# likojack/bnv_fusion

Hardware: AMD Instinct MI355X
Metric: depth frames/sec fused+decoded, 640x480 @ 256^3 grid (higher is better)
Workload: dtype f32 operands split into f16 hi+lo, 3 products on v_mfma_f32_16x16x32_f16, f32 accumulate

## Files before the change

### bnv_fusion_amd/csrc/encode.hip

```cpp
#include <stddef.h>

#include <atomic>
#include <utility>
#include <vector>

#include "frontend.hpp"
#include "tcnn_mlp.hpp"

namespace bnv {

int g_num_cus = 0;
int g_last_hip_error = 0;
std::atomic<int> g_reserve_cus{0};
std::atomic<int> g_finalize_blocks{0};
std::atomic<int> g_tcnn_shared_table{1};
std::atomic<int> g_tcnn_block_encoder{1};
std::atomic<int> g_mlp_mode{1};

bool g_prof_on = false;
static std::vector<std::pair<hipEvent_t, hipEvent_t>> g_prof_events[PROF_KINDS];
static size_t g_prof_used[PROF_KINDS] = {0, 0, 0, 0};

void prof_mark(int kind, bool begin, hipStream_t stream) {
  auto& ring = g_prof_events[kind];
// ... 651 lines not shown
  const int64_t n = ctl->n_deferred;
  const int nyz = g.n_xyz[1] * g.n_xyz[2];
  for (int64_t q = (int64_t)blockIdx.x * 256 + threadIdx.x; q < n; q += (int64_t)gridDim.x * 256) {
    const int id = ids[defer_list[q]];
    const int x = id / nyz, r = id - x * nyz, y = r / g.n_xyz[2], z = r - y * g.n_xyz[2];
    if (shard_is_boundary(x, y, z, g)) atomicAdd(&s_hist[voxel_owner(x, y, z, g) & 63], 1);
  }
  __syncthreads();
  if (threadIdx.x < 64 && threadIdx.x < g.shard_world && s_hist[threadIdx.x])
    atomicAdd(&ctl->shard_boundary[threadIdx.x], s_hist[threadIdx.x]);
}

struct ValidFlags {
  const int32_t* counts;
  const int32_t* ids;
  bnv_grid_t g;
  int emit_all;
  __device__ uint32_t operator()(int64_t s) const {
    if (!emit_all && counts[s] < g.min_pts_in_grid) return 0;
    if (g.shard_world > 1) {
      const int id = ids[s];
      const int nyz = g.n_xyz[1] * g.n_xyz[2];
      const int x = id / nyz, r = id - x * nyz, y = r / g.n_xyz[2], z = r - y * g.n_xyz[2];
      if (voxel_owner(x, y, z, g) != g.shard_rank) return 0;
    }
    return 1;
  }
};

struct PairTiles {
  const int32_t* list;
  int n_pairs, n_points, n_pblocks, n_tiles;
};
__device__ __forceinline__ PairTiles pair_tiles(int n_points, const int32_t* __restrict__ pair_list,
                                                const int32_t* __restrict__ n_pairs) {
  PairTiles T;
  T.list = pair_list;
  T.n_points = n_points;
  T.n_pblocks = (n_points + 31) >> 5;
  T.n_pairs = pair_list ? *n_pairs : 0;
  T.n_tiles = pair_list ? (T.n_pairs + 31) >> 5 : T.n_pblocks * 8;
  return T;
}
__device__ __forceinline__ bool tile_pair(const PairTiles& T, int t, int j, int* i, int* k) {
  if (T.list) {
    const int e = t * 32 + j;
    if (e >= T.n_pairs) return false;
    const int p = T.list[e];
    *i = p >> 3;
    *k = p & 7;
    return true;
  }
  *k = t / T.n_pblocks;
  *i = (t - *k * T.n_pblocks) * 32 + j;
  return *i < T.n_points;
}

__device__ __forceinline__ f32x16 relu16(f32x16 v) {
#pragma unroll
  for (int r = 0; r < 16; ++r) v[r] = relu_bits(v[r]);
  return v;
}

__device__ __forceinline__ f32x16 bias_init(const float* __restrict__ b, int mb, int h) {
  f32x16 v;
#pragma unroll
  for (int q = 0; q < 4; ++q) {
    const f32x4 t = *(const f32x4*)&b[mb * 32 + 8 * q + 4 * h];
#pragma unroll
    for (int i = 0; i < 4; ++i) v[4 * q + i] = t[i];
  }
  return v;
}

__device__ __forceinline__ void layer128(const float* __restrict__ wp, const float* __restrict__ bias,
                                         const f32x16 (&in)[4], f32x16 (&out)[4], int lane, int h) {
#pragma unroll
  for (int mb = 0; mb < 4; ++mb) out[mb] = bias_init(bias, mb, h);
#pragma unroll
  for (int nb = 0; nb < 4; ++nb) {
#pragma unroll
    for (int rq = 0; rq < 4; ++rq) {
      f32x4 a[4];
#pragma unroll
      for (int mb = 0; mb < 4; ++mb)
        a[mb] = *(const f32x4*)&wp[(((mb * 4 + nb) * 4 + rq) * 64 + lane) * 4];
#pragma unroll
// ... 50 lines not shown
    if (s > 0) v[q] -= ((unsigned long long)phi << 32) | plo;
  }
}

__device__ __forceinline__ void scatter_tile(const f32x16& o, int slot, int j, int h, int32_t* __restrict__ counts,
                                             long long* __restrict__ acc) {
  unsigned long long v[4];
  bool is_end;
  int len;
  tile_run_sums(o, slot, j, h, v, is_end, len);
#ifdef BNV_PROBE_NO_SCATTER
  if ((blockIdx.x & 63) != 0) return;
#endif
  if (slot >= 0 && is_end) {
    unsigned long long* dst = (unsigned long long*)acc + ((uint32_t)slot * 8u + 4u * (uint32_t)h);
#pragma unroll
    for (int q = 0; q < 4; ++q) atomicAdd(dst + q, v[q]);
    if (h == 0) atomicAdd(&counts[slot], len);
  }
}

__global__ __launch_bounds__(512, 2) void k_pointnet_scatter(
    const float* __restrict__ pts, int n_points, bnv_grid_t g, const float* __restrict__ wpack,
    const uint32_t* __restrict__ bitmap, const uint32_t* __restrict__ word_prefix,
    int32_t* __restrict__ counts, long long* __restrict__ acc, const int32_t* __restrict__ pair_list,
    const int32_t* __restrict__ n_pairs) {
  extern __shared__ __attribute__((aligned(16))) float lds[];
  stage_to_lds<512>(wpack, lds, PN_TOTAL * 4);
  __syncthreads();

  const int lane = threadIdx.x & 63;
  const int wave = __builtin_amdgcn_readfirstlane(threadIdx.x >> 6);
  const int j = lane & 31, h = lane >> 5;
  const PairTiles T = pair_tiles(n_points, pair_list, n_pairs);
  const int n_tiles = T.n_tiles;
  const int nyz = g.n_xyz[1] * g.n_xyz[2];

  for (int t = blockIdx.x * 8 + wave; t < n_tiles; t += gridDim.x * 8) {
    int i = 0, k = 0;
    const bool have = tile_pair(T, t, j, &i, &k);
    float in0 = 0.f, in1 = 0.f, in2 = 0.f;
    int slot = -1;
    bool valid = false;
    if (have) {
      const float* p = pts + (size_t)i * 6;
      const float x = p[0], y = p[1], z = p[2];
      valid = in_bounds(x, y, z, g);
      if (valid) {
        const float xn = voxel_coord(x, g.bound_min[0], g.voxel_size);
        const float yn = voxel_coord(y, g.bound_min[1], g.voxel_size);
        const float zn = voxel_coord(z, g.bound_min[2], g.voxel_size);
        const int gx = (k & 1) ? (int)ceilf(xn) : (int)floorf(xn);
        const int gy = (k & 2) ? (int)ceilf(yn) : (int)floorf(yn);
        const int gz = (k & 4) ? (int)ceilf(zn) : (int)floorf(zn);
        if (voxel_owner(gx, gy, gz, g) == g.shard_rank) {
          const uint32_t id = (uint32_t)(gx * nyz + gy * g.n_xyz[2] + gz);
          const uint32_t word = bitmap[id >> 5];
          slot = (int)(word_prefix[id >> 5] + __popc(word & ((1u << (id & 31)) - 1u)));
        }
        const float rx = relative_coord(xn, gx, g.voxel_size);
        const float ry = relative_coord(yn, gy, g.voxel_size);
        const float rz = relative_coord(zn, gz, g.voxel_size);
        in0 = h ? ry : rx;
        in1 = h ? p[3] : rz;
        in2 = h ? p[5] : p[4];
      }
    }
    if (__ballot(slot >= 0) == 0ULL) continue;

    f32x16 ha[4], hb[4];
#pragma unroll
    for (int mb = 0; mb < 4; ++mb) ha[mb] = bias_init(lds + PN_B1, mb, h);
    {
// ... 12 lines not shown
#pragma unroll
    for (int mb = 0; mb < 4; ++mb) hb[mb] = relu16(hb[mb]);
    layer128(lds + PN_W3, lds + PN_B3, hb, ha, lane, h);
#pragma unroll
    for (int mb = 0; mb < 4; ++mb) ha[mb] = relu16(ha[mb]);
    f32x16 o;
#pragma unroll
    for (int r = 0; r < 16; ++r) o[r] = 0.f;
    {
      const f32x4 b4 = *(const f32x4*)&lds[PN_B4 + 4 * h];
#pragma unroll
      for (int r = 0; r < 4; ++r) o[r] = b4[r];
    }
#pragma unroll
    for (int nb = 0; nb < 4; ++nb) {
#pragma unroll
      for (int rq = 0; rq < 4; ++rq) {
        f32x4 a = {0.f, 0.f, 0.f, 0.f};
        if (j < 8) a = *(const f32x4*)&lds[PN_W4 + ((((nb * 4 + rq) * 2 + h) * 8) + j) * 4];
#pragma unroll
        for (int i = 0; i < 4; ++i)
          o = __builtin_amdgcn_mfma_f32_32x32x2f32(a[i], ha[nb][4 * rq + i], o, 0, 0, 0);
      }
    }
    scatter_tile(o, slot, j, h, counts, acc);
  }
}


typedef __attribute__((address_space(3))) const half8 lds_half8_t;
typedef __attribute__((address_space(3))) const f32x4 lds_f32x4_t;
constexpr int kLdsWin = 61440;

#ifdef BNV_PHASE_PROF
__device__ unsigned long long g_enc_phase[8 * 16];
#define BNV_EPH(i)                                                                          \
  do {                                                                                      \
    if ((threadIdx.x & 63) == 0) {                                                          \
      unsigned long long* _p = (unsigned long long*)((char*)lds + PX_LDS_BYTES) + (threadIdx.x >> 6) * 16; \
      const unsigned long long _t = clock64();                                              \
      _p[i] += _t - _p[15];                                                                 \
      _p[15] = _t;                                                                          \
    }                                                                                       \
  } while (0)
constexpr int kEncProfLds = 8 * 16 * 8;
#else
#define BNV_EPH(i)
constexpr int kEncProfLds = 0;
#endif

struct EncLdsX {
  uint32_t w[3];
  uint32_t b;
};
__device__ __forceinline__ half8 ldsx_wfrag(const EncLdsX& L, int byte_off) {
  const int b = byte_off / kLdsWin;
  return *(lds_half8_t*)((b == 0 ? L.w[0] : (b == 1 ? L.w[1] : L.w[2])) + (uint32_t)(byte_off - b * kLdsWin));
}
__device__ __forceinline__ f32x4 ldsx_bias(const EncLdsX& L, int layer, int rb) {
  return *(lds_f32x4_t*)(L.b + (uint32_t)((layer * 128 + rb * 16) * 4));
}

template <int NPROD>
__device__ __forceinline__ void layer128_x(const EncLdsX& L, int w_off, int layer, const half8 (&inh)[4][2],
                                           const half8 (&inl)[4][2], f32x4 (&out)[8][2]) {
#pragma unroll
  for (int rb = 0; rb < 8; ++rb) out[rb][0] = out[rb][1] = ldsx_bias(L, layer, rb);
  half8 ah[2], al[2];
#define BNV_LOAD_WX(q)                                                        \
  {                                                                           \
    const int wb = (w_off + (q) * 2 * 64 * 8) * 2;                            \
    ah[(q) & 1] = ldsx_wfrag(L, wb);                                          \
    if (NPROD == 3) al[(q) & 1] = ldsx_wfrag(L, wb + 1024);                   \
  }
  BNV_LOAD_WX(0);
#pragma unroll
  for (int q = 0; q < 32; ++q) {
    if (q + 1 < 32) BNV_LOAD_WX(q + 1);
    __builtin_amdgcn_sched_barrier(0);
    const int s = q >> 3, rb = q & 7;
    if constexpr (NPROD == 3) {
      out[rb][0] = __builtin_amdgcn_mfma_f32_16x16x32_f16(al[q & 1], inh[s][0], out[rb][0], 0, 0, 0);
      out[rb][1] = __builtin_amdgcn_mfma_f32_16x16x32_f16(al[q & 1], inh[s][1], out[rb][1], 0, 0, 0);
      out[rb][0] = __builtin_amdgcn_mfma_f32_16x16x32_f16(ah[q & 1], inl[s][0], out[rb][0], 0, 0, 0);
      out[rb][1] = __builtin_amdgcn_mfma_f32_16x16x32_f16(ah[q & 1], inl[s][1], out[rb][1], 0, 0, 0);
    }
    out[rb][0] = __builtin_amdgcn_mfma_f32_16x16x32_f16(ah[q & 1], inh[s][0], out[rb][0], 0, 0, 0);
    out[rb][1] = __builtin_amdgcn_mfma_f32_16x16x32_f16(ah[q & 1], inh[s][1], out[rb][1], 0, 0, 0);
    __builtin_amdgcn_sched_barrier(0);
  }
#undef BNV_LOAD_WX
}

template <int NPROD>
__device__ __forceinline__ void split_x(const f32x4 (&acc)[8][2], half8 (&oh)[4][2], half8 (&ol)[4][2]) {
#pragma unroll
  for (int s = 0; s < 4; ++s)
#pragma unroll
    for (int cb = 0; cb < 2; ++cb) {
      float x[8];
#pragma unroll
      for (int e = 0; e < 8; ++e) x[e] = relu_bits(acc[2 * s + (e >> 2)][cb][e & 3]);
      if (NPROD == 3) {
        split8_f16(x, oh[s][cb], ol[s][cb]);
      } else {
#pragma unroll
        for (int e = 0; e < 8; ++e) oh[s][cb][e] = (_Float16)x[e];
      }
    }
}

__device__ __forceinline__ void scatter_tile_x(const f32x4& o, int slot, int n, int g, int32_t* __restrict__ counts,
                                               long long* __restrict__ acc) {
  uint32_t lo[4], hi[4];
#pragma unroll
  for (int q = 0; q < 4; ++q) {
    const float r = __builtin_rintf(o[q] * kFixedScale);
    const float hf = __builtin_floorf(r * (1.0f / kFixedScale));
    hi[q] = (uint32_t)(int)hf;
    lo[q] = (uint32_t)__builtin_fmaf(hf, -kFixedScale, r);
  }
#define BNV_SCAN_STEP(ctrl)                                                      \
  "v_add_co_u32_dpp %0, vcc, %0, %0 " ctrl "\n"                                  \
  "v_addc_co_u32_dpp %1, vcc, %1, %1, vcc " ctrl "\n"                            \
  "v_add_co_u32_dpp %2, vcc, %2, %2 " ctrl "\n"                                  \
  "v_addc_co_u32_dpp %3, vcc, %3, %3, vcc " ctrl "\n"                            \
  "v_add_co_u32_dpp %4, vcc, %4, %4 " ctrl "\n"                                  \
  "v_addc_co_u32_dpp %5, vcc, %5, %5, vcc " ctrl "\n"                            \
  "v_add_co_u32_dpp %6, vcc, %6, %6 " ctrl "\n"                                  \
  "v_addc_co_u32_dpp %7, vcc, %7, %7, vcc " ctrl "\n"
  asm volatile("s_nop 1\n"
               BNV_SCAN_STEP("row_shr:1 row_mask:0xf bank_mask:0xf bound_ctrl:1")
               BNV_SCAN_STEP("row_shr:2 row_mask:0xf bank_mask:0xf bound_ctrl:1")
               BNV_SCAN_STEP("row_shr:4 row_mask:0xf bank_mask:0xf bound_ctrl:1")
               BNV_SCAN_STEP("row_shr:8 row_mask:0xf bank_mask:0xf bound_ctrl:1")
               : "+v"(lo[0]), "+v"(hi[0]), "+v"(lo[1]), "+v"(hi[1]), "+v"(lo[2]), "+v"(hi[2]), "+v"(lo[3]), "+v"(hi[3])
               :
               : "vcc");
#undef BNV_SCAN_STEP
  {
    const int tsrc = ((g & 1) * 16 + 15) * 4;
#pragma unroll
    for (int q = 0; q < 4; ++q) {
      const uint32_t tl = (uint32_t)__builtin_amdgcn_ds_bpermute(tsrc, (int)lo[q]);
      const uint32_t th = (uint32_t)__builtin_amdgcn_ds_bpermute(tsrc, (int)hi[q]);
      if (g >= 2) {
        const unsigned long long v = (((unsigned long long)hi[q] << 32) | lo[q]) + (((unsigned long long)th << 32) | tl);
        lo[q] = (uint32_t)v;
        hi[q] = (uint32_t)(v >> 32);
      }
    }
  }
  const int p = (g >> 1) * 16 + n;
  const int slot15 = __builtin_amdgcn_readlane(slot, 15);
  const int prev_row = __builtin_amdgcn_update_dpp(0, slot, 0x111 , 0xf, 0xf, false);
  const int prev = n == 0 ? slot15 : prev_row;
  const unsigned long long heads64 = __ballot(p == 0 || prev != slot);
  const uint32_t heads = ((uint32_t)heads64 & 0xffffu) | (((uint32_t)(heads64 >> 32) & 0xffffu) << 16);
  const int s = 31 - __clz((int)(heads & (0xffffffffu >> (31 - p))));
  const bool is_end = p == 31 || ((heads >> (p + 1)) & 1u);
  const int sp = s > 0 ? s - 1 : 0;
  const int src = (((sp >> 4) * 2 + (g & 1)) * 16 + (sp & 15)) * 4;
  uint32_t plo[4], phi[4];
#pragma unroll
  for (int q = 0; q < 4; ++q) {
    plo[q] = (uint32_t)__builtin_amdgcn_ds_bpermute(src, (int)lo[q]);
    phi[q] = (uint32_t)__builtin_amdgcn_ds_bpermute(src, (int)hi[q]);
  }
#ifdef BNV_PROBE_NO_SCATTER
  if ((blockIdx.x & 63) != 0) return;
#endif
  if (slot >= 0 && is_end) {
    unsigned long long* dst = (unsigned long long*)acc + ((uint32_t)slot * 8u + 4u * (uint32_t)(g & 1));
#pragma unroll
    for (int q = 0; q < 4; ++q) {
      unsigned long long v = ((unsigned long long)hi[q] << 32) | lo[q];
      if (s > 0) v -= ((unsigned long long)phi[q] << 32) | plo[q];
      atomicAdd(dst + q, v);
    }
    if ((g & 1) == 0) atomicAdd(&counts[slot], p - s + 1);
  }
}

template <int NPROD>
__global__ __launch_bounds__(512, 2) __attribute__((amdgpu_num_vgpr(120))) void k_pointnet_scatter_x(
    const float* __restrict__ pts, int n_points, bnv_grid_t g, const float* __restrict__ wpack,
    const uint32_t* __restrict__ bitmap, const uint32_t* __restrict__ word_prefix,
    int32_t* __restrict__ counts, long long* __restrict__ acc, int32_t* __restrict__ error,
    const int32_t* __restrict__ pair_list, const int32_t* __restrict__ n_pairs) {
  extern __shared__ __attribute__((aligned(16))) float lds[];
  const float n_cert = wpack[PN_CERT];
  float* lb = lds + PX_TOTAL / 2;
  for (int i = threadIdx.x; i < 128 * 3 + 8; i += 512) lb[i] = wpack[PN_B1 + i];
  stage_to_lds<512>(wpack + PX_OFF, lds, PX_TOTAL * 2);
  int* tile_ctr = (int*)((char*)lds + PX_TOTAL * 2 + (128 * 3 + 8) * 4);
  if (threadIdx.x == 0) *tile_ctr = 0;
  __syncthreads();

  const int lane = threadIdx.x & 63;
  const int n = lane & 15, gk = lane >> 4;
  const int pair = (gk >> 1) * 16 + n;
  const PairTiles T = pair_tiles(n_points, pair_list, n_pairs);
  const int n_tiles = T.n_tiles;
  const int nyz = g.n_xyz[1] * g.n_xyz[2];
  EncLdsX L;
  {
    const uint32_t lds0 = (uint32_t)(uintptr_t)(__attribute__((address_space(3))) float*)lds;
    L.w[0] = lds0 + lane * 16;
    L.w[1] = L.w[0] + kLdsWin;
    L.w[2] = L.w[0] + 2 * kLdsWin;
    L.b = lds0 + PX_TOTAL * 2 + gk * 16;
    asm volatile("" : "+v"(L.w[0]), "+v"(L.w[1]), "+v"(L.w[2]), "+v"(L.b));
  }

  const int tstep = gridDim.x * 8;
  auto grab = [&]() -> int {
    int c = 0;
    if (lane == 0) c = atomicAdd(tile_ctr, 1);
    c = __builtin_amdgcn_readfirstlane(c);
    return blockIdx.x * 8 + (c & 7) + (c >> 3) * tstep;
  };
  float raw[6];
  int raw_k = 0;
  bool raw_ok = false;
  float nin[6];
  uint32_t n_id = 0, n_word = 0, n_pref = 0;
  bool n_own = false;
  auto stage1 = [&](int t) {
    raw_ok = false;
    if (t < n_tiles) {
      int i = 0;
      if (tile_pair(T, t, pair, &i, &raw_k)) {
        const float* p = pts + (size_t)i * 6;
#pragma unroll
        for (int c = 0; c < 6; ++c) raw[c] = p[c];
        raw_ok = true;
      }
    }
  };
  auto stage2 = [&](int t) {
    n_own = false;
#pragma unroll
    for (int c = 0; c < 6; ++c) nin[c] = 0.f;
    if (raw_ok && in_bounds(raw[0], raw[1], raw[2], g)) {
      const int k = raw_k;
      const float xn = voxel_coord(raw[0], g.bound_min[0], g.voxel_size);
      const float yn = voxel_coord(raw[1], g.bound_min[1], g.voxel_size);
      const float zn = voxel_coord(raw[2], g.bound_min[2], g.voxel_size);
      const int gx = (k & 1) ? (int)ceilf(xn) : (int)floorf(xn);
      const int gy = (k & 2) ? (int)ceilf(yn) : (int)floorf(yn);
      const int gz = (k & 4) ? (int)ceilf(zn) : (int)floorf(zn);
      if (voxel_owner(gx, gy, gz, g) == g.shard_rank) {
        n_own = true;
        n_id = (uint32_t)(gx * nyz + gy * g.n_xyz[2] + gz);
        n_word = bitmap[n_id >> 5];
        n_pref = word_prefix[n_id >> 5];
      }
      if ((gk & 1) == 0) {
        nin[0] = relative_coord(xn, gx, g.voxel_size);
        nin[1] = relative_coord(yn, gy, g.voxel_size);
        nin[2] = relative_coord(zn, gz, g.voxel_size);
        nin[3] = raw[3];
        nin[4] = raw[4];
        nin[5] = raw[5];
      }
      if (!(fmaxf(fmaxf(fabsf(raw[3]), fabsf(raw[4])), fabsf(raw[5])) <= n_cert)) *error = 3;
    }
  };
  int t = grab();
  stage1(t);
  stage2(t);
  int t_next = grab(), t_next2 = 0;
  stage1(t_next);
#ifdef BNV_PHASE_PROF
  if ((threadIdx.x & 63) < 16)
    ((unsigned long long*)((char*)lds + PX_LDS_BYTES))[(threadIdx.x >> 6) * 16 + (threadIdx.x & 63)] = 0;
  if ((threadIdx.x & 63) == 0) ((unsigned long long*)((char*)lds + PX_LDS_BYTES))[(threadIdx.x >> 6) * 16 + 15] = clock64();
#endif

  for (; t < n_tiles; t = t_next, t_next = t_next2) {
    float in[6];
#pragma unroll
    for (int c = 0; c < 6; ++c) in[c] = nin[c];
    const int slot = n_own ? (int)(n_pref + __popc(n_word & ((1u << (n_id & 31)) - 1u))) : -1;
    stage2(t_next);
    t_next2 = grab();
    stage1(t_next2);
    __builtin_amdgcn_sched_barrier(0);
    BNV_EPH(0);
    if (__ballot(slot >= 0) == 0ULL) continue;

    f32x4 ha[8][2], hb[8][2];
    {
      half8 bh[2], bl[2];
#pragma unroll
      for (int cb = 0; cb < 2; ++cb) {
        float x[8];
#pragma unroll
        for (int e = 0; e < 8; ++e) x[e] = 0.f;
#pragma unroll
        for (int e = 0; e < 6; ++e) {
          const float other = __shfl(in[e], (lane + 32) & 63, 64);
          x[e] = gk == 0 ? (cb == 0 ? in[e] : other) : 0.f;
        }
        if (NPROD == 3) {
          split8_f16(x, bh[cb], bl[cb]);
        } else {
#pragma unroll
          for (int e = 0; e < 8; ++e) bh[cb][e] = (_Float16)x[e];
        }
      }
#pragma unroll
      for (int rb = 0; rb < 8; ++rb) {
        const half8 ahi = ldsx_wfrag(L, (PX_W1 + rb * 2 * 64 * 8) * 2), alo = ldsx_wfrag(L, (PX_W1 + rb * 2 * 64 * 8) * 2 + 1024);
        const f32x4 b = ldsx_bias(L, 0, rb);
#pragma unroll
        for (int cb = 0; cb < 2; ++cb) {
          f32x4 c = b;
          if constexpr (NPROD == 3) {
            c = __builtin_amdgcn_mfma_f32_16x16x32_f16(alo, bh[cb], c, 0, 0, 0);
            c = __builtin_amdgcn_mfma_f32_16x16x32_f16(ahi, bl[cb], c, 0, 0, 0);
          }
          ha[rb][cb] = __builtin_amdgcn_mfma_f32_16x16x32_f16(ahi, bh[cb], c, 0, 0, 0);
        }
      }
    }
    BNV_EPH(1);
    half8 sh[4][2], sl[4][2];
    split_x<NPROD>(ha, sh, sl);
    BNV_EPH(2);
    layer128_x<NPROD>(L, PX_W2, 1, sh, sl, hb);
    BNV_EPH(3);
    split_x<NPROD>(hb, sh, sl);
    BNV_EPH(4);
    layer128_x<NPROD>(L, PX_W3, 2, sh, sl, ha);
    BNV_EPH(5);
    split_x<NPROD>(ha, sh, sl);
    BNV_EPH(6);
    f32x4 o[2];
    o[0] = o[1] = *(lds_f32x4_t*)(L.b + 384 * 4);
    {
      half8 w4h[4], w4l[4];
      __builtin_amdgcn_sched_barrier(0);
#pragma unroll
      for (int s = 0; s < 4; ++s) {
        w4h[s] = ldsx_wfrag(L, (PX_W4 + s * 2 * 64 * 8) * 2);
        if (NPROD == 3) w4l[s] = ldsx_wfrag(L, (PX_W4 + s * 2 * 64 * 8) * 2 + 1024);
      }
#pragma unroll
      for (int s = 0; s < 4; ++s) {
#pragma unroll
        for (int cb = 0; cb < 2; ++cb) {
          if constexpr (NPROD == 3) {
            o[cb] = __builtin_amdgcn_mfma_f32_16x16x32_f16(w4l[s], sh[s][cb], o[cb], 0, 0, 0);
            o[cb] = __builtin_amdgcn_mfma_f32_16x16x32_f16(w4h[s], sl[s][cb], o[cb], 0, 0, 0);
          }
          o[cb] = __builtin_amdgcn_mfma_f32_16x16x32_f16(w4h[s], sh[s][cb], o[cb], 0, 0, 0);
        }
      }
    }
    f32x4 mine;
#pragma unroll
    for (int i = 0; i < 4; ++i) {
      const float other = __shfl(o[1][i], (lane + 32) & 63, 64);
      mine[i] = gk < 2 ? o[0][i] : other;
    }
    BNV_EPH(7);
    scatter_tile_x(mine, slot, n, gk, counts, acc);
    BNV_EPH(8);
  }
#ifdef BNV_PHASE_PROF
  if ((threadIdx.x & 63) < 15)
    atomicAdd(&g_enc_phase[(threadIdx.x >> 6) * 16 + (threadIdx.x & 63)],
              ((unsigned long long*)((char*)lds + PX_LDS_BYTES))[(threadIdx.x >> 6) * 16 + (threadIdx.x & 63)]);
#endif
}

typedef TcnnPack<1> PointPack;

__global__ __launch_bounds__(256) void k_pointnet_scatter_t(
    const float* __restrict__ pts, int n_points, bnv_grid_t g, const float* __restrict__ wpack,
    const uint32_t* __restrict__ bitmap, const uint32_t* __restrict__ word_prefix,
    int32_t* __restrict__ counts, long long* __restrict__ acc, const int32_t* __restrict__ pair_list,
    const int32_t* __restrict__ n_pairs) {
  __shared__ __attribute__((aligned(16))) _Float16 wh[PointPack::TOTAL];
  stage_to_lds<256>(wpack, wh, PointPack::TOTAL * 2);
  __syncthreads();
  const int lane = threadIdx.x & 63;
  const int wave = __builtin_amdgcn_readfirstlane(threadIdx.x >> 6);
  const int j = lane & 31, h = lane >> 5;
  const PairTiles T = pair_tiles(n_points, pair_list, n_pairs);
  const int n_tiles = T.n_tiles;
  const int nyz = g.n_xyz[1] * g.n_xyz[2];
  for (int t = blockIdx.x * 4 + wave; t < n_tiles; t += gridDim.x * 4) {
    int i = 0, k = 0;
    const bool have = tile_pair(T, t, j, &i, &k);
    half8 b;
#pragma unroll
    for (int e = 0; e < 8; ++e) b[e] = (_Float16)1.0f;
    int slot = -1;
    bool valid = false;
    if (have) {
      const float* p = pts + (size_t)i * 6;
      const float x = p[0], y = p[1], z = p[2];
      if (in_bounds(x, y, z, g)) {
        valid = true;
        const float xn = voxel_coord(x, g.bound_min[0], g.voxel_size);
        const float yn = voxel_coord(y, g.bound_min[1], g.voxel_size);
        const float zn = voxel_coord(z, g.bound_min[2], g.voxel_size);
        const int gx = (k & 1) ? (int)ceilf(xn) : (int)floorf(xn);
        const int gy = (k & 2) ? (int)ceilf(yn) : (int)floorf(yn);
        const int gz = (k & 4) ? (int)ceilf(zn) : (int)floorf(zn);
        if (voxel_owner(gx, gy, gz, g) == g.shard_rank) {
          const uint32_t id = (uint32_t)(gx * nyz + gy * g.n_xyz[2] + gz);
          const uint32_t word = bitmap[id >> 5];
          slot = (int)(word_prefix[id >> 5] + __popc(word & ((1u << (id & 31)) - 1u)));
        }
        if (h == 0) {
          b[0] = (_Float16)relative_coord(xn, gx, g.voxel_size);
          b[1] = (_Float16)relative_coord(yn, gy, g.voxel_size);
          b[2] = (_Float16)relative_coord(zn, gz, g.voxel_size);
          b[3] = (_Float16)p[3];
        } else {
          b[0] = (_Float16)p[4];
          b[1] = (_Float16)p[5];
        }
      }
    }
    if (__ballot(slot >= 0) == 0ULL) continue;
// ... 288 lines not shown
  if (bound_mask) bound_mask[i] = in_bounds(x, y, z, g) ? 1 : 0;
  const float xn = voxel_coord(x, g.bound_min[0], g.voxel_size);
  const float yn = voxel_coord(y, g.bound_min[1], g.voxel_size);
  const float zn = voxel_coord(z, g.bound_min[2], g.voxel_size);
  const int nyz = g.n_xyz[1] * g.n_xyz[2];
#pragma unroll
  for (int k = 0; k < 8; ++k) {
    const int cb = kCornerCeilBits[k];
    const int gx = (cb & 1) ? (int)ceilf(xn) : (int)floorf(xn);
    const int gy = (cb & 2) ? (int)ceilf(yn) : (int)floorf(yn);
    const int gz = (cb & 4) ? (int)ceilf(zn) : (int)floorf(zn);
    const size_t p = (size_t)k * n_points + i;
    if (grid_ids) {
      grid_ids[p * 3 + 0] = gx;
      grid_ids[p * 3 + 1] = gy;
      grid_ids[p * 3 + 2] = gz;
    }
    if (flat_ids) flat_ids[p] = (int64_t)(gx * nyz + gy * g.n_xyz[2] + gz);
    if (rel_xyz) {
      rel_xyz[p * 3 + 0] = __fmul_rn(__fsub_rn(xn, (float)gx), g.voxel_size);
      rel_xyz[p * 3 + 1] = __fmul_rn(__fsub_rn(yn, (float)gy), g.voxel_size);
      rel_xyz[p * 3 + 2] = __fmul_rn(__fsub_rn(zn, (float)gz), g.voxel_size);
    }
  }
}

}

using namespace bnv;

extern "C" {

#ifdef BNV_PHASE_PROF
int bnv_dev_enc_phase_read(unsigned long long* out128) {
  BNV_HIP_CHECK(hipDeviceSynchronize());
  BNV_HIP_CHECK(hipMemcpyFromSymbol(out128, HIP_SYMBOL(bnv::g_enc_phase), 128 * sizeof(unsigned long long)));
  unsigned long long z[128] = {};
  BNV_HIP_CHECK(hipMemcpyToSymbol(HIP_SYMBOL(bnv::g_enc_phase), z, sizeof(z)));
  return BNV_OK;
}
#endif


int bnv_init(int device) {
  BNV_HIP_CHECK(hipSetDevice(device));
  int cus = 0;
  BNV_HIP_CHECK(hipDeviceGetAttribute(&cus, hipDeviceAttributeMultiprocessorCount, device));
  g_num_cus = cus;
  BNV_HIP_CHECK(hipFuncSetAttribute((const void*)k_pointnet_scatter,
                                    hipFuncAttributeMaxDynamicSharedMemorySize, PN_TOTAL * 4));
  BNV_HIP_CHECK(hipFuncSetAttribute((const void*)k_pointnet_scatter_x<3>,
                                    hipFuncAttributeMaxDynamicSharedMemorySize, PX_LDS_BYTES + kEncProfLds));
  BNV_HIP_CHECK(hipFuncSetAttribute((const void*)k_pointnet_scatter_x<1>,
                                    hipFuncAttributeMaxDynamicSharedMemorySize, PX_LDS_BYTES + kEncProfLds));
  extern int bnv_decode_init();
  return bnv_decode_init();
}

int bnv_num_compute_units(void) { return g_num_cus; }
int bnv_last_hip_error(void) { return g_last_hip_error; }

const char* bnv_status_string(int s) {
  switch (s) {
    case BNV_OK: return "ok";
    case BNV_ERR_INVALID_ARGUMENT: return "invalid argument";
    case BNV_ERR_WORKSPACE_TOO_SMALL: return "workspace too small";
    case BNV_ERR_HIP: return "HIP runtime error";
    case BNV_ERR_NOT_INITIALISED: return "bnv_init not called";
    case BNV_ERR_CAPACITY: return "capacity exceeded";
    default: return "unknown";
// ... 168 lines not shown
                               int64_t out_capacity, int emit_all, bnv_encode_counters_t* counters,
                               int max_workgroups, bnv_stream_t stream_) {
  return bnv_encode_finish_image_parts(input_pts, n_points, image_width, grid_host, pointnet_pack, ws_ptr, ws_bytes,
                                       ws_max_points, out_feats, out_pcounts, out_flat_ids, out_grid_ids, out_capacity,
                                       emit_all, counters, max_workgroups, 3, stream_);
}

int bnv_encode_finish_image_parts(const float* input_pts, int64_t n_points, int image_width,
                                  const bnv_grid_t* grid_host, const float* pointnet_pack, void* ws_ptr,
                                  size_t ws_bytes, int64_t ws_max_points, float* out_feats, int64_t* out_pcounts,
                                  int64_t* out_flat_ids, int64_t* out_grid_ids, int64_t out_capacity, int emit_all,
                                  bnv_encode_counters_t* counters, int max_workgroups, int parts,
                                  bnv_stream_t stream_) {
  if (g_num_cus <= 0) return BNV_ERR_NOT_INITIALISED;
  if (image_width < 0 || max_workgroups < 0 || parts < 1 || parts > 3) return BNV_ERR_INVALID_ARGUMENT;
  if (!input_pts || !grid_host || !pointnet_pack || !ws_ptr || !counters || n_points < 0 ||
      n_points > (1 << 27) || ws_max_points < n_points)
    return BNV_ERR_INVALID_ARGUMENT;
  const bnv_grid_t g = *grid_host;
  if (!grid_ok(g)) return BNV_ERR_INVALID_ARGUMENT;
  hipStream_t stream = (hipStream_t)stream_;
  EncodeWs ws;
  if (encode_ws_layout(ws_max_points, g.n_xyz, (char*)ws_ptr, &ws) > ws_bytes) return BNV_ERR_WORKSPACE_TOO_SMALL;
  if (n_points == 0) {
    if (parts & 2) BNV_HIP_CHECK(hipMemsetAsync(counters, 0, sizeof(bnv_encode_counters_t), stream));
    return BNV_OK;
  }
  const int n = (int)n_points;
  const int n_tiles = ((n + 31) / 32) * 8;
  const int reserve = g_reserve_cus.load(std::memory_order_relaxed);
  int grid_pn = g_num_cus - reserve > 0 ? g_num_cus - reserve : 1;
  if (max_workgroups > 0 && grid_pn > max_workgroups) grid_pn = max_workgroups;
  if (grid_pn > (n_tiles + 7) / 8) grid_pn = (n_tiles + 7) / 8;
  const int mlp = mlp_mode_of(g.mlp_mode);
  const int32_t* plist = (g.shard_world > 1 && !tcnn_blocks(g)) ? ws.pair_list : (const int32_t*)nullptr;
  if (parts & 1) {
    ProfScope prof(PROF_POINTNET, stream);
    if (tcnn_blocks(g)) {
      const int n_blocks = (n + 31) / 32 + 64;
      const int n_units = (n_blocks + kTbWaves - 1) / kTbWaves + 64;
      const int cus_tb = max_workgroups > 0 && max_workgroups < g_num_cus ? max_workgroups : g_num_cus;
      const int grid_tb = cus_tb * 2 < n_units ? cus_tb * 2 : n_units;
      auto kern = g_tcnn_shared_table.load(std::memory_order_relaxed) ? k_pointnet_scatter_tb<true> : k_pointnet_scatter_tb<false>;
      hipLaunchKernelGGL(kern, dim3(grid_tb), dim3(64 * kTbWaves), 0, stream, input_pts, n, image_width, g,
                         pointnet_pack, ws.bitmap, ws.word_prefix, ws.counts, ws.acc);
    } else if (mlp == 2)
      hipLaunchKernelGGL(k_pointnet_scatter_t, dim3(g_num_cus * 4 < (n_tiles + 3) / 4 ? g_num_cus * 4 : (n_tiles + 3) / 4),
                         dim3(256), 0, stream, input_pts, n, g, pointnet_pack, ws.bitmap, ws.word_prefix, ws.counts,
                         ws.acc, plist, &ws.ctl->n_pairs);
    else if (mlp == 1) {
      hipLaunchKernelGGL((k_pointnet_scatter_x<3>), dim3(grid_pn), dim3(512), PX_LDS_BYTES + kEncProfLds, stream,
                         input_pts, n, g, pointnet_pack, ws.bitmap, ws.word_prefix, ws.counts, ws.acc, &ws.ctl->error,
                         plist, &ws.ctl->n_pairs);
    } else if (mlp == 3) {
      hipLaunchKernelGGL((k_pointnet_scatter_x<1>), dim3(grid_pn), dim3(512), PX_LDS_BYTES + kEncProfLds, stream,
                         input_pts, n, g, pointnet_pack, ws.bitmap, ws.word_prefix, ws.counts, ws.acc, &ws.ctl->error,
                         plist, &ws.ctl->n_pairs);
    } else
      hipLaunchKernelGGL(k_pointnet_scatter, dim3(grid_pn), dim3(512), PN_TOTAL * 4, stream, input_pts, n, g,
                         pointnet_pack, ws.bitmap, ws.word_prefix, ws.counts, ws.acc, plist, &ws.ctl->n_pairs);
  }
  BNV_LAUNCH_CHECK();
  if (!(parts & 2)) return BNV_OK;
  const int nb_max = (int)((ws.max_unique + kFinTile - 1) / kFinTile);
  const int nb_res = 2 * g_num_cus;
  const int nb_opt = g_finalize_blocks.load(std::memory_order_relaxed);
  const int nb_cap = nb_opt > 0 && nb_opt < nb_res ? nb_opt : nb_res;
  const int nb_u = nb_max < nb_cap ? nb_max : nb_cap;
  hipLaunchKernelGGL(k_finalize, dim3(nb_u), dim3(kFinTile), 0, stream, g, emit_all, ws.bitmap, ws.ids,
                     ws.counts, ws.acc, ws.tile_state, next_epoch(), ws.ctl, ws.valid_blocks, (n + 255) / 256, out_feats,
                     out_pcounts, out_flat_ids, out_grid_ids, out_capacity, counters);
  BNV_LAUNCH_CHECK();
  return BNV_OK;
}

int bnv_encode_pointcloud(const float* input_pts, int64_t n_points, const bnv_grid_t* grid_host,
                          const float* pointnet_pack, void* ws_ptr, size_t ws_bytes, int64_t ws_max_points,
                          float* out_feats,
                          int64_t* out_pcounts, int64_t* out_flat_ids, int64_t* out_grid_ids,
                          int64_t out_capacity, int emit_all, bnv_encode_counters_t* counters,
                          bnv_stream_t stream) {
  if (!pointnet_pack || !counters) return BNV_ERR_INVALID_ARGUMENT;
  const int rc = bnv_encode_begin(input_pts, n_points, grid_host, ws_ptr, ws_bytes, ws_max_points, stream);
  if (rc != BNV_OK) return rc;
  return bnv_encode_finish(input_pts, n_points, grid_host, pointnet_pack, ws_ptr, ws_bytes, ws_max_points, out_feats,
                           out_pcounts, out_flat_ids, out_grid_ids, out_capacity, emit_all, counters, stream);
}

// ... 14 lines not shown
```

Measured before the change: 551.0.

## Shrink pointnet MFMA tile to 16 points with 16 waves and a weight ring

The mixed-precision pointnet encoder now processes 16 points per wave tile instead of 32, which halves the accumulator and activation register arrays. It launches 16 waves per workgroup instead of 8 and drops the fixed VGPR cap. All four layers' weight fragments are streamed through a 4-deep register ring that spans layer boundaries, and the segmented scatter reduction is simplified to a single 16-lane row. The aim is more resident waves to hide LDS and MFMA latency, at the cost of more tile-loop and atomic overhead per point and wasted lanes in the point-staging stage.

```diff
diff --git a/bnv_fusion_amd/csrc/encode.hip b/bnv_fusion_amd/csrc/encode.hip
--- a/bnv_fusion_amd/csrc/encode.hip
+++ b/bnv_fusion_amd/csrc/encode.hip
@@ -707,19 +707,21 @@
   const int32_t* list;
   int n_pairs, n_points, n_pblocks, n_tiles;
 };
+template <int W>
 __device__ __forceinline__ PairTiles pair_tiles(int n_points, const int32_t* __restrict__ pair_list,
                                                 const int32_t* __restrict__ n_pairs) {
   PairTiles T;
   T.list = pair_list;
   T.n_points = n_points;
-  T.n_pblocks = (n_points + 31) >> 5;
+  T.n_pblocks = (n_points + W - 1) / W;
   T.n_pairs = pair_list ? *n_pairs : 0;
-  T.n_tiles = pair_list ? (T.n_pairs + 31) >> 5 : T.n_pblocks * 8;
+  T.n_tiles = pair_list ? (T.n_pairs + W - 1) / W : T.n_pblocks * 8;
   return T;
 }
+template <int W>
 __device__ __forceinline__ bool tile_pair(const PairTiles& T, int t, int j, int* i, int* k) {
   if (T.list) {
-    const int e = t * 32 + j;
+    const int e = t * W + j;
     if (e >= T.n_pairs) return false;
     const int p = T.list[e];
     *i = p >> 3;
@@ -727,7 +729,7 @@
     return true;
   }
   *k = t / T.n_pblocks;
-  *i = (t - *k * T.n_pblocks) * 32 + j;
+  *i = (t - *k * T.n_pblocks) * W + j;
   return *i < T.n_points;
 }
 
@@ -844,13 +846,13 @@
   const int lane = threadIdx.x & 63;
   const int wave = __builtin_amdgcn_readfirstlane(threadIdx.x >> 6);
   const int j = lane & 31, h = lane >> 5;
-  const PairTiles T = pair_tiles(n_points, pair_list, n_pairs);
+  const PairTiles T = pair_tiles<32>(n_points, pair_list, n_pairs);
   const int n_tiles = T.n_tiles;
   const int nyz = g.n_xyz[1] * g.n_xyz[2];
 
   for (int t = blockIdx.x * 8 + wave; t < n_tiles; t += gridDim.x * 8) {
     int i = 0, k = 0;
-    const bool have = tile_pair(T, t, j, &i, &k);
+    const bool have = tile_pair<32>(T, t, j, &i, &k);
     float in0 = 0.f, in1 = 0.f, in2 = 0.f;
     int slot = -1;
     bool valid = false;
@@ -929,8 +931,11 @@
 typedef __attribute__((address_space(3))) const f32x4 lds_f32x4_t;
 constexpr int kLdsWin = 61440;
 
+constexpr int kXWaves = 16;
+constexpr int kXTile = 16;
+
 #ifdef BNV_PHASE_PROF
-__device__ unsigned long long g_enc_phase[8 * 16];
+__device__ unsigned long long g_enc_phase[kXWaves * 16];
 #define BNV_EPH(i)                                                                          \
   do {                                                                                      \
     if ((threadIdx.x & 63) == 0) {                                                          \
@@ -940,7 +945,7 @@
       _p[15] = _t;                                                                          \
     }                                                                                       \
   } while (0)
-constexpr int kEncProfLds = 8 * 16 * 8;
+constexpr int kEncProfLds = kXWaves * 16 * 8;
 #else
 #define BNV_EPH(i)
 constexpr int kEncProfLds = 0;
@@ -958,53 +963,57 @@
   return *(lds_f32x4_t*)(L.b + (uint32_t)((layer * 128 + rb * 16) * 4));
 }
 
+constexpr int kXStepHalves = 2 * 64 * 8;
+constexpr int kXSteps = PX_TOTAL / kXStepHalves;
+constexpr int kXRing = 4;
+static_assert(PX_W1 == 0 && PX_W2 == 8 * kXStepHalves && PX_W3 == 40 * kXStepHalves && PX_W4 == 72 * kXStepHalves &&
+                  kXSteps == 76,
+              "the four layers' fragments are one contiguous stream of steps");
+struct EncRingX {
+  half8 h[kXRing], l[kXRing];
+};
 template <int NPROD>
-__device__ __forceinline__ void layer128_x(const EncLdsX& L, int w_off, int layer, const half8 (&inh)[4][2],
-                                           const half8 (&inl)[4][2], f32x4 (&out)[8][2]) {
-#pragma unroll
-  for (int rb = 0; rb < 8; ++rb) out[rb][0] = out[rb][1] = ldsx_bias(L, layer, rb);
-  half8 ah[2], al[2];
-#define BNV_LOAD_WX(q)                                                        \
-  {                                                                           \
-    const int wb = (w_off + (q) * 2 * 64 * 8) * 2;                            \
-    ah[(q) & 1] = ldsx_wfrag(L, wb);                                          \
-    if (NPROD == 3) al[(q) & 1] = ldsx_wfrag(L, wb + 1024);                   \
-  }
-  BNV_LOAD_WX(0);
-#pragma unroll
-  for (int q = 0; q < 32; ++q) {
-    if (q + 1 < 32) BNV_LOAD_WX(q + 1);
-    __builtin_amdgcn_sched_barrier(0);
-    const int s = q >> 3, rb = q & 7;
-    if constexpr (NPROD == 3) {
-      out[rb][0] = __builtin_amdgcn_mfma_f32_16x16x32_f16(al[q & 1], inh[s][0], out[rb][0], 0, 0, 0);
-      out[rb][1] = __builtin_amdgcn_mfma_f32_16x16x32_f16(al[q & 1], inh[s][1], out[rb][1], 0, 0, 0);
-      out[rb][0] = __builtin_amdgcn_mfma_f32_16x16x32_f16(ah[q & 1], inl[s][0], out[rb][0], 0, 0, 0);
-      out[rb][1] = __builtin_amdgcn_mfma_f32_16x16x32_f16(ah[q & 1], inl[s][1], out[rb][1], 0, 0, 0);
-    }
-    out[rb][0] = __builtin_amdgcn_mfma_f32_16x16x32_f16(ah[q & 1], inh[s][0], out[rb][0], 0, 0, 0);
-    out[rb][1] = __builtin_amdgcn_mfma_f32_16x16x32_f16(ah[q & 1], inh[s][1], out[rb][1], 0, 0, 0);
-    __builtin_amdgcn_sched_barrier(0);
-  }
-#undef BNV_LOAD_WX
-}
-
+__device__ __forceinline__ void ringx_load(const EncLdsX& L, EncRingX& R, int u) {
+  if (u >= kXSteps) return;
+  R.h[u % kXRing] = ldsx_wfrag(L, u * kXStepHalves * 2);
+  if (NPROD == 3) R.l[u % kXRing] = ldsx_wfrag(L, u * kXStepHalves * 2 + 1024);
+}
 template <int NPROD>
-__device__ __forceinline__ void split_x(const f32x4 (&acc)[8][2], half8 (&oh)[4][2], half8 (&ol)[4][2]) {
-#pragma unroll
-  for (int s = 0; s < 4; ++s)
-#pragma unroll
-    for (int cb = 0; cb < 2; ++cb) {
-      float x[8];
-#pragma unroll
-      for (int e = 0; e < 8; ++e) x[e] = relu_bits(acc[2 * s + (e >> 2)][cb][e & 3]);
-      if (NPROD == 3) {
-        split8_f16(x, oh[s][cb], ol[s][cb]);
-      } else {
-#pragma unroll
-        for (int e = 0; e < 8; ++e) oh[s][cb][e] = (_Float16)x[e];
-      }
-    }
+__device__ __forceinline__ void ringx_step(const EncLdsX& L, EncRingX& R, int u, const half8& inh, const half8& inl,
+                                           f32x4& c) {
+  ringx_load<NPROD>(L, R, u + kXRing - 1);
+  __builtin_amdgcn_sched_barrier(0);
+  if constexpr (NPROD == 3) {
+    c = __builtin_amdgcn_mfma_f32_16x16x32_f16(R.l[u % kXRing], inh, c, 0, 0, 0);
+    c = __builtin_amdgcn_mfma_f32_16x16x32_f16(R.h[u % kXRing], inl, c, 0, 0, 0);
+  }
+  c = __builtin_amdgcn_mfma_f32_16x16x32_f16(R.h[u % kXRing], inh, c, 0, 0, 0);
+  __builtin_amdgcn_sched_barrier(0);
+}
+
+template <int NPROD>
+__device__ __forceinline__ void layer128_x(const EncLdsX& L, EncRingX& R, int u0, int layer, const half8 (&inh)[4],
+                                           const half8 (&inl)[4], f32x4 (&out)[8]) {
+#pragma unroll
+  for (int rb = 0; rb < 8; ++rb) out[rb] = ldsx_bias(L, layer, rb);
+#pragma unroll
+  for (int q = 0; q < 32; ++q) ringx_step<NPROD>(L, R, u0 + q, inh[q >> 3], inl[q >> 3], out[q & 7]);
+}
+
+template <int NPROD>
+__device__ __forceinline__ void split_x(const f32x4 (&acc)[8], half8 (&oh)[4], half8 (&ol)[4]) {
+#pragma unroll
+  for (int s = 0; s < 4; ++s) {
+    float x[8];
+#pragma unroll
+    for (int e = 0; e < 8; ++e) x[e] = relu_bits(acc[2 * s + (e >> 2)][e & 3]);
+    if (NPROD == 3) {
+      split8_f16(x, oh[s], ol[s]);
+    } else {
+#pragma unroll
+      for (int e = 0; e < 8; ++e) oh[s][e] = (_Float16)x[e];
+    }
+  }
 }
 
 __device__ __forceinline__ void scatter_tile_x(const f32x4& o, int slot, int n, int g, int32_t* __restrict__ counts,
@@ -1035,29 +1044,12 @@
                :
                : "vcc");
 #undef BNV_SCAN_STEP
-  {
-    const int tsrc = ((g & 1) * 16 + 15) * 4;
-#pragma unroll
-    for (int q = 0; q < 4; ++q) {
-      const uint32_t tl = (uint32_t)__builtin_amdgcn_ds_bpermute(tsrc, (int)lo[q]);
-      const uint32_t th = (uint32_t)__builtin_amdgcn_ds_bpermute(tsrc, (int)hi[q]);
-      if (g >= 2) {
-        const unsigned long long v = (((unsigned long long)hi[q] << 32) | lo[q]) + (((unsigned long long)th << 32) | tl);
-        lo[q] = (uint32_t)v;
-        hi[q] = (uint32_t)(v >> 32);
-      }
-    }
-  }
-  const int p = (g >> 1) * 16 + n;
-  const int slot15 = __builtin_amdgcn_readlane(slot, 15);
-  const int prev_row = __builtin_amdgcn_update_dpp(0, slot, 0x111 , 0xf, 0xf, false);
-  const int prev = n == 0 ? slot15 : prev_row;
-  const unsigned long long heads64 = __ballot(p == 0 || prev != slot);
-  const uint32_t heads = ((uint32_t)heads64 & 0xffffu) | (((uint32_t)(heads64 >> 32) & 0xffffu) << 16);
-  const int s = 31 - __clz((int)(heads & (0xffffffffu >> (31 - p))));
-  const bool is_end = p == 31 || ((heads >> (p + 1)) & 1u);
+  const int prev = __builtin_amdgcn_update_dpp(0, slot, 0x111 , 0xf, 0xf, false);
+  const uint32_t heads = (uint32_t)__ballot(n == 0 || prev != slot) & 0xffffu;
+  const int s = 31 - __clz((int)(heads & (0xffffu >> (15 - n))));
+  const bool is_end = n == 15 || ((heads >> (n + 1)) & 1u);
   const int sp = s > 0 ? s - 1 : 0;
-  const int src = (((sp >> 4) * 2 + (g & 1)) * 16 + (sp & 15)) * 4;
+  const int src = ((g & 1) * 16 + sp) * 4;
   uint32_t plo[4], phi[4];
 #pragma unroll
   for (int q = 0; q < 4; ++q) {
@@ -1075,12 +1067,12 @@
       if (s > 0) v -= ((unsigned long long)phi[q] << 32) | plo[q];
       atomicAdd(dst + q, v);
     }
-    if ((g & 1) == 0) atomicAdd(&counts[slot], p - s + 1);
+    if (g == 0) atomicAdd(&counts[slot], n - s + 1);
   }
 }
 
 template <int NPROD>
-__global__ __launch_bounds__(512, 2) __attribute__((amdgpu_num_vgpr(120))) void k_pointnet_scatter_x(
+__global__ __launch_bounds__(64 * kXWaves) void k_pointnet_scatter_x(
     const float* __restrict__ pts, int n_points, bnv_grid_t g, const float* __restrict__ wpack,
     const uint32_t* __restrict__ bitmap, const uint32_t* __restrict__ word_prefix,
     int32_t* __restrict__ counts, long long* __restrict__ acc, int32_t* __restrict__ error,
@@ -1088,16 +1080,16 @@
   extern __shared__ __attribute__((aligned(16))) float lds[];
   const float n_cert = wpack[PN_CERT];
   float* lb = lds + PX_TOTAL / 2;
-  for (int i = threadIdx.x; i < 128 * 3 + 8; i += 512) lb[i] = wpack[PN_B1 + i];
-  stage_to_lds<512>(wpack + PX_OFF, lds, PX_TOTAL * 2);
+  for (int i = threadIdx.x; i < 128 * 3 + 8; i += 64 * kXWaves) lb[i] = wpack[PN_B1 + i];
+  stage_to_lds<64 * kXWaves>(wpack + PX_OFF, lds, PX_TOTAL * 2);
   int* tile_ctr = (int*)((char*)lds + PX_TOTAL * 2 + (128 * 3 + 8) * 4);
   if (threadIdx.x == 0) *tile_ctr = 0;
   __syncthreads();
 
   const int lane = threadIdx.x & 63;
   const int n = lane & 15, gk = lane >> 4;
-  const int pair = (gk >> 1) * 16 + n;
-  const PairTiles T = pair_tiles(n_points, pair_list, n_pairs);
+  const bool stager = gk < 2;
+  const PairTiles T = pair_tiles<kXTile>(n_points, pair_list, n_pairs);
   const int n_tiles = T.n_tiles;
   const int nyz = g.n_xyz[1] * g.n_xyz[2];
   EncLdsX L;
@@ -1110,12 +1102,12 @@
     asm volatile("" : "+v"(L.w[0]), "+v"(L.w[1]), "+v"(L.w[2]), "+v"(L.b));
   }
 
-  const int tstep = gridDim.x * 8;
+  const int tstep = gridDim.x * kXWaves;
   auto grab = [&]() -> int {
     int c = 0;
     if (lane == 0) c = atomicAdd(tile_ctr, 1);
     c = __builtin_amdgcn_readfirstlane(c);
-    return blockIdx.x * 8 + (c & 7) + (c >> 3) * tstep;
+    return blockIdx.x * kXWaves + (c & (kXWaves - 1)) + (int)((unsigned)c / kXWaves) * tstep;
   };
   float raw[6];
   int raw_k = 0;
@@ -1125,9 +1117,9 @@
   bool n_own = false;
   auto stage1 = [&](int t) {
     raw_ok = false;
-    if (t < n_tiles) {
+    if (stager && t < n_tiles) {
       int i = 0;
-      if (tile_pair(T, t, pair, &i, &raw_k)) {
+      if (tile_pair<kXTile>(T, t, n, &i, &raw_k)) {
         const float* p = pts + (size_t)i * 6;
 #pragma unroll
         for (int c = 0; c < 6; ++c) raw[c] = p[c];
@@ -1153,7 +1145,7 @@
         n_word = bitmap[n_id >> 5];
         n_pref = word_prefix[n_id >> 5];
       }
-      if ((gk & 1) == 0) {
+      if (gk == 0) {
         nin[0] = relative_coord(xn, gx, g.voxel_size);
         nin[1] = relative_coord(yn, gy, g.voxel_size);
         nin[2] = relative_coord(zn, gz, g.voxel_size);
@@ -1187,83 +1179,43 @@
     BNV_EPH(0);
     if (__ballot(slot >= 0) == 0ULL) continue;
 
-    f32x4 ha[8][2], hb[8][2];
+    EncRingX R;
+#pragma unroll
+    for (int u = 0; u < kXRing - 1; ++u) ringx_load<NPROD>(L, R, u);
+    f32x4 ha[8], hb[8];
     {
-      half8 bh[2], bl[2];
-#pragma unroll
-      for (int cb = 0; cb < 2; ++cb) {
-        float x[8];
-#pragma unroll
-        for (int e = 0; e < 8; ++e) x[e] = 0.f;
-#pragma unroll
-        for (int e = 0; e < 6; ++e) {
-          const float other = __shfl(in[e], (lane + 32) & 63, 64);
-          x[e] = gk == 0 ? (cb == 0 ? in[e] : other) : 0.f;
-        }
-        if (NPROD == 3) {
-          split8_f16(x, bh[cb], bl[cb]);
-        } else {
-#pragma unroll
-          for (int e = 0; e < 8; ++e) bh[cb][e] = (_Float16)x[e];
-        }
-      }
-#pragma unroll
-      for (int rb = 0; rb < 8; ++rb) {
-        const half8 ahi = ldsx_wfrag(L, (PX_W1 + rb * 2 * 64 * 8) * 2), alo = ldsx_wfrag(L, (PX_W1 + rb * 2 * 64 * 8) * 2 + 1024);
-        const f32x4 b = ldsx_bias(L, 0, rb);
-#pragma unroll
-        for (int cb = 0; cb < 2; ++cb) {
-          f32x4 c = b;
-          if constexpr (NPROD == 3) {
-            c = __builtin_amdgcn_mfma_f32_16x16x32_f16(alo, bh[cb], c, 0, 0, 0);
-            c = __builtin_amdgcn_mfma_f32_16x16x32_f16(ahi, bl[cb], c, 0, 0, 0);
-          }
-          ha[rb][cb] = __builtin_amdgcn_mfma_f32_16x16x32_f16(ahi, bh[cb], c, 0, 0, 0);
-        }
-      }
+      half8 bh, bl;
+      float x[8];
+#pragma unroll
+      for (int e = 0; e < 8; ++e) x[e] = e < 6 ? in[e] : 0.f;
+      if (NPROD == 3) {
+        split8_f16(x, bh, bl);
+      } else {
+#pragma unroll
+        for (int e = 0; e < 8; ++e) bh[e] = (_Float16)x[e];
+      }
+#pragma unroll
+      for (int rb = 0; rb < 8; ++rb) ha[rb] = ldsx_bias(L, 0, rb);
+#pragma unroll
+      for (int rb = 0; rb < 8; ++rb) ringx_step<NPROD>(L, R, rb, bh, bl, ha[rb]);
     }
     BNV_EPH(1);
-    half8 sh[4][2], sl[4][2];
+    half8 sh[4], sl[4];
     split_x<NPROD>(ha, sh, sl);
     BNV_EPH(2);
-    layer128_x<NPROD>(L, PX_W2, 1, sh, sl, hb);
+    layer128_x<NPROD>(L, R, 8, 1, sh, sl, hb);
     BNV_EPH(3);
     split_x<NPROD>(hb, sh, sl);
     BNV_EPH(4);
-    layer128_x<NPROD>(L, PX_W3, 2, sh, sl, ha);
+    layer128_x<NPROD>(L, R, 40, 2, sh, sl, ha);
     BNV_EPH(5);
     split_x<NPROD>(ha, sh, sl);
     BNV_EPH(6);
-    f32x4 o[2];
-    o[0] = o[1] = *(lds_f32x4_t*)(L.b + 384 * 4);
-    {
-      half8 w4h[4], w4l[4];
-      __builtin_amdgcn_sched_barrier(0);
-#pragma unroll
-      for (int s = 0; s < 4; ++s) {
-        w4h[s] = ldsx_wfrag(L, (PX_W4 + s * 2 * 64 * 8) * 2);
-        if (NPROD == 3) w4l[s] = ldsx_wfrag(L, (PX_W4 + s * 2 * 64 * 8) * 2 + 1024);
-      }
-#pragma unroll
-      for (int s = 0; s < 4; ++s) {
-#pragma unroll
-        for (int cb = 0; cb < 2; ++cb) {
-          if constexpr (NPROD == 3) {
-            o[cb] = __builtin_amdgcn_mfma_f32_16x16x32_f16(w4l[s], sh[s][cb], o[cb], 0, 0, 0);
-            o[cb] = __builtin_amdgcn_mfma_f32_16x16x32_f16(w4h[s], sl[s][cb], o[cb], 0, 0, 0);
-          }
-          o[cb] = __builtin_amdgcn_mfma_f32_16x16x32_f16(w4h[s], sh[s][cb], o[cb], 0, 0, 0);
-        }
-      }
-    }
-    f32x4 mine;
-#pragma unroll
-    for (int i = 0; i < 4; ++i) {
-      const float other = __shfl(o[1][i], (lane + 32) & 63, 64);
-      mine[i] = gk < 2 ? o[0][i] : other;
-    }
+    f32x4 o = *(lds_f32x4_t*)(L.b + 384 * 4);
+#pragma unroll
+    for (int s = 0; s < 4; ++s) ringx_step<NPROD>(L, R, 72 + s, sh[s], sl[s], o);
     BNV_EPH(7);
-    scatter_tile_x(mine, slot, n, gk, counts, acc);
+    scatter_tile_x(o, slot, n, gk, counts, acc);
     BNV_EPH(8);
   }
 #ifdef BNV_PHASE_PROF
@@ -1286,12 +1238,12 @@
   const int lane = threadIdx.x & 63;
   const int wave = __builtin_amdgcn_readfirstlane(threadIdx.x >> 6);
   const int j = lane & 31, h = lane >> 5;
-  const PairTiles T = pair_tiles(n_points, pair_list, n_pairs);
+  const PairTiles T = pair_tiles<32>(n_points, pair_list, n_pairs);
   const int n_tiles = T.n_tiles;
   const int nyz = g.n_xyz[1] * g.n_xyz[2];
   for (int t = blockIdx.x * 4 + wave; t < n_tiles; t += gridDim.x * 4) {
     int i = 0, k = 0;
-    const bool have = tile_pair(T, t, j, &i, &k);
+    const bool have = tile_pair<32>(T, t, j, &i, &k);
     half8 b;
 #pragma unroll
     for (int e = 0; e < 8; ++e) b[e] = (_Float16)1.0f;
@@ -1646,10 +1598,10 @@
 extern "C" {
 
 #ifdef BNV_PHASE_PROF
-int bnv_dev_enc_phase_read(unsigned long long* out128) {
+int bnv_dev_enc_phase_read(unsigned long long* out256) {
   BNV_HIP_CHECK(hipDeviceSynchronize());
-  BNV_HIP_CHECK(hipMemcpyFromSymbol(out128, HIP_SYMBOL(bnv::g_enc_phase), 128 * sizeof(unsigned long long)));
-  unsigned long long z[128] = {};
+  BNV_HIP_CHECK(hipMemcpyFromSymbol(out256, HIP_SYMBOL(bnv::g_enc_phase), 256 * sizeof(unsigned long long)));
+  unsigned long long z[256] = {};
   BNV_HIP_CHECK(hipMemcpyToSymbol(HIP_SYMBOL(bnv::g_enc_phase), z, sizeof(z)));
   return BNV_OK;
 }
@@ -1884,6 +1836,10 @@
   int grid_pn = g_num_cus - reserve > 0 ? g_num_cus - reserve : 1;
   if (max_workgroups > 0 && grid_pn > max_workgroups) grid_pn = max_workgroups;
   if (grid_pn > (n_tiles + 7) / 8) grid_pn = (n_tiles + 7) / 8;
+  const int n_tiles_x = ((n + kXTile - 1) / kXTile) * 8;
+  int grid_px = g_num_cus - reserve > 0 ? g_num_cus - reserve : 1;
+  if (max_workgroups > 0 && grid_px > max_workgroups) grid_px = max_workgroups;
+  if (grid_px > (n_tiles_x + kXWaves - 1) / kXWaves) grid_px = (n_tiles_x + kXWaves - 1) / kXWaves;
   const int mlp = mlp_mode_of(g.mlp_mode);
   const int32_t* plist = (g.shard_world > 1 && !tcnn_blocks(g)) ? ws.pair_list : (const int32_t*)nullptr;
   if (parts & 1) {
@@ -1901,11 +1857,11 @@
                          dim3(256), 0, stream, input_pts, n, g, pointnet_pack, ws.bitmap, ws.word_prefix, ws.counts,
                          ws.acc, plist, &ws.ctl->n_pairs);
     else if (mlp == 1) {
-      hipLaunchKernelGGL((k_pointnet_scatter_x<3>), dim3(grid_pn), dim3(512), PX_LDS_BYTES + kEncProfLds, stream,
+      hipLaunchKernelGGL((k_pointnet_scatter_x<3>), dim3(grid_px), dim3(64 * kXWaves), PX_LDS_BYTES + kEncProfLds, stream,
                          input_pts, n, g, pointnet_pack, ws.bitmap, ws.word_prefix, ws.counts, ws.acc, &ws.ctl->error,
                          plist, &ws.ctl->n_pairs);
     } else if (mlp == 3) {
-      hipLaunchKernelGGL((k_pointnet_scatter_x<1>), dim3(grid_pn), dim3(512), PX_LDS_BYTES + kEncProfLds, stream,
+      hipLaunchKernelGGL((k_pointnet_scatter_x<1>), dim3(grid_px), dim3(64 * kXWaves), PX_LDS_BYTES + kEncProfLds, stream,
                          input_pts, n, g, pointnet_pack, ws.bitmap, ws.word_prefix, ws.counts, ws.acc, &ws.ctl->error,
                          plist, &ws.ctl->n_pairs);
     } else
```

Result: slower. 544.4 (-1.2%).
